# cvsp-lab/ICLR2025_3D-MOM

Hardware: AMD Instinct MI355X
Metric: 4DGS train-steps/sec @200k Gaussians, 960×540, 60 frames; render FPS (higher is better)
Workload: dtype f32; 1 GPU; 200k Gaussians, 60 frames, 960x540, HexPlane on; gaussians=200000, frames=60, width=960, height=540, parallelism=single, ranks_seen=1, gaussians_at_end=200000, steps_replayed_after_overflow=0

## Files before the change

### iclr2025_3d-mom_amd/_native.py

```python
from __future__ import annotations

import ctypes as C
import os
import subprocess

_HERE = os.path.dirname(os.path.abspath(__file__))
LIB_PATH = os.environ.get("MOM4D_LIB") or os.path.join(_HERE, "lib", "libmom4d.so")
_lib = None

MOM_OK, MOM_EINVAL, MOM_ELAUNCH, MOM_ECAPACITY, MOM_EUNAVAILABLE = 0, -1, -2, -3, -4
_ERR = {MOM_EINVAL: "invalid argument", MOM_ELAUNCH: "HIP launch/runtime failure", MOM_ECAPACITY: "scratch too small",
        MOM_EUNAVAILABLE: "run-time dependency missing (librccl)"}
COMM_F32, COMM_I32, COMM_SUM, COMM_MAX = 0, 1, 0, 1


class MomError(RuntimeError):
    pass


GACC_FLOATS = int(os.environ.get("MOM_GACC_FLOATS", "12"))
ABI_VERSION = 8


class MomRasterArgs(C.Structure):
# ... 198 lines not shown
    lib.mom_ssim_forward.argtypes = [i32, i32, i32, vp, vp, vp, vp, vp, vp]
    lib.mom_ssim_forward_slab.argtypes = [i32, i32, i32, sz, i32, i32, i32, i32, vp, vp, vp, vp, vp, vp]
    lib.mom_ssim_backward_slab.argtypes = [i32, i32, i32, sz, vp, vp, vp, vp, C.c_float, vp, vp, vp]
    lib.mom_ssim_backward.argtypes = [i32, i32, i32, vp, vp, vp, vp, C.c_float, vp, vp, vp]
    lib.mom_activations_forward.argtypes = [i32, vp, vp, vp, vp, vp, vp, vp]
    lib.mom_activations_backward.argtypes = [i32, vp, vp, vp, vp, vp, vp, vp, vp, vp, vp]
    lib.mom_image_to_rgb8.argtypes = [i32, i32, i32, vp, vp, vp]
    lib.mom_png_bound.restype = sz
    lib.mom_png_bound.argtypes = [i32, i32, i32]
    lib.mom_png_scratch_bytes.restype = sz
    lib.mom_png_scratch_bytes.argtypes = [i32, i32, i32]
    lib.mom_png_encode.argtypes = [i32, i32, i32, vp, vp, sz, vp, vp, vp]
    lib.mom_png_encode_host.argtypes = [i32, i32, i32, vp, vp, sz, vp]
    lib.mom_png_tables.argtypes = [i32, vp, vp, vp, i32, vp]
    lib.mom_profile_enable.argtypes = [i32, i32]
    lib.mom_profile_read.argtypes = [i32, C.POINTER(C.c_double), C.POINTER(C.c_longlong), i32]
    lib.mom_profile_name.restype = C.c_char_p
    lib.mom_profile_name.argtypes = [i32]
    lib.mom_knn_scratch_bytes.restype = sz
    lib.mom_knn_scratch_bytes.argtypes = [i32]
    lib.mom_knn_mean_dist2.argtypes = [i32, vp, vp, vp, vp]
    return lib


SSIM_SUM_SLOTS = 64
SELECT_MAX_TENSORS = 32


class MomRowSelect(C.Structure):
    _fields_ = [("src", C.c_void_p), ("dst", C.c_void_p), ("row_bytes", C.c_uint)]
# ... 13 lines not shown
    "mom_raster_forward_geometry", "mom_raster_forward_render", "mom_raster_backward", "mom_mark_visible",
    "mom_selftest_wave_sum", "mom_selftest_row_reduce", "mom_hexplane_forward", "mom_hexplane_backward", "mom_hexplane_backward_lines", "mom_adam_step", "mom_l1_loss",
    "mom_plane_regulation", "mom_knn_scratch_bytes", "mom_knn_mean_dist2",
    "mom_profile_enable", "mom_profile_read", "mom_profile_name",
    "mom_morton_order_scratch_bytes", "mom_morton_order", "mom_activations_forward", "mom_activations_backward", "mom_deform_forward", "mom_deform_forward_activated", "mom_deform_backward_scratch_bytes", "mom_deform_backward", "mom_deform_backward_split",
    "mom_ssim_forward", "mom_ssim_backward", "mom_raster_backward_render", "mom_raster_backward_geometry",
    "mom_densify_stats", "mom_select_scratch_bytes", "mom_select_plan", "mom_select_apply",
    "mom_ssim_forward_slab", "mom_ssim_backward_slab",
    "mom_hexplane_backward_scratch_bytes", "mom_hexplane_orders_scratch_bytes", "mom_hexplane_orders", "mom_image_to_rgb8",
    "mom_l1_loss_acc", "mom_plane_regulation_acc", "mom_plane_regulation_grad",
    "mom_deform_field_supported", "mom_deform_field_scratch_bytes", "mom_deform_field_forward",
    "mom_stream_wait_stream", "mom_stream_mark", "mom_stream_wait_mark", "mom_zero_async",
    "mom_comm_available", "mom_comm_last_error", "mom_comm_unique_id", "mom_comm_create", "mom_comm_destroy", "mom_comm_abort",
    "mom_comm_world", "mom_comm_rank", "mom_comm_group_start", "mom_comm_group_end", "mom_comm_all_reduce", "mom_comm_all_gather",
    "mom_comm_reduce_scatter",
    "mom_raster_backward_acc", "mom_raster_backward_geometry_acc",
    "mom_deform_forward_n", "mom_deform_forward_activated_n", "mom_deform_backward_n", "mom_deform_backward_split_n",
    "mom_deform_field16_supported", "mom_deform_field16_scratch_bytes", "mom_deform_field16_forward",
    "mom_densify_scratch_bytes", "mom_densify_plan", "mom_densify_apply",
    "mom_sceneflow_fit_scratch_bytes", "mom_sceneflow_fit", "mom_flow_sample",
    "mom_png_bound", "mom_png_scratch_bytes", "mom_png_encode", "mom_png_encode_host", "mom_png_tables",
]


ABI_STRUCTS = None


def _abi_structs():
    return [("MOM_STRUCT_RASTER_ARGS", MomRasterArgs), ("MOM_STRUCT_RASTER_GRADS", MomRasterGrads),
            ("MOM_STRUCT_RASTER_LAYOUT", MomRasterLayout), ("MOM_STRUCT_HEXPLANE", MomHexPlane),
            ("MOM_STRUCT_ADAM_TENSOR", MomAdamTensor), ("MOM_STRUCT_ROW_SELECT", MomRowSelect),
# ... 74 lines not shown
```

### iclr2025_3d-mom_amd/csrc/mom_common.h

```cpp
#pragma once
#include <hip/hip_runtime.h>
#include <stdint.h>
#include <stddef.h>
#include <stdlib.h>
#include "../../include/mom4d.h"

#define MOM_WAVE 64
#define MOM_ALIGN 256

struct GeomView {
    float4* rec;
    float* cov3D;
    uchar4* clamped;
    float* gacc;
    unsigned long long* reach;
};
struct ImageView {
    uint32_t* hdr;
    uint32_t* tile_counts;
    uint32_t* tile_cursor;
    uint2* ranges;
    uint32_t* n_contrib;
    float* final_T;
    uint32_t* tile_order;
};
struct BinView {
    uint64_t* keys;
    uint32_t* point_list;
};

static inline size_t mom_align_up(size_t x) { return (x + MOM_ALIGN - 1) & ~(size_t)(MOM_ALIGN - 1); }

static inline size_t geom_view(char* base, int P, GeomView* v)
{
    size_t off = 0;
    size_t o_rec = off; off = mom_align_up(off + (size_t)P * 48);
    size_t o_cov = off; off = mom_align_up(off + (size_t)P * 24);
    size_t o_cl = off; off = mom_align_up(off + (size_t)P * 4);
    size_t o_ga = off; off = mom_align_up(off + (size_t)P * MOM_GACC_FLOATS * 4);
// ... 7 lines not shown
    }
    return off + MOM_ALIGN;
}
static inline size_t image_view(char* base, int W, int H, ImageView* v)
{
    const size_t tiles = (size_t)((W + MOM_TILE - 1) / MOM_TILE) * ((H + MOM_TILE - 1) / MOM_TILE);
    const size_t N = (size_t)W * H;
    size_t off = 0;
    size_t o_h = off; off = mom_align_up(off + 64 * 4);
    size_t o_c = off; off = mom_align_up(off + tiles * 4);
    size_t o_u = off; off = mom_align_up(off + tiles * 4);
    size_t o_r = off; off = mom_align_up(off + tiles * 8);
    size_t o_n = off; off = mom_align_up(off + N * 4);
    size_t o_t = off; off = mom_align_up(off + N * 4);
    size_t o_o = off; off = mom_align_up(off + tiles * 4);
    if (v) {
        v->tile_order = (uint32_t*)(base + o_o);
        v->hdr = (uint32_t*)(base + o_h);
        v->tile_counts = (uint32_t*)(base + o_c);
        v->tile_cursor = (uint32_t*)(base + o_u);
        v->ranges = (uint2*)(base + o_r);
        v->n_contrib = (uint32_t*)(base + o_n);
        v->final_T = (float*)(base + o_t);
    }
    return off + MOM_ALIGN;
}
static inline size_t bin_view(char* base, size_t cap, BinView* v)
{
    size_t off = 0;
    size_t o_p = off; off = mom_align_up(off + cap * 4);
    size_t o_k = off; off = mom_align_up(off + cap * 8);
    if (v) {
// ... 117 lines not shown
```

### iclr2025_3d-mom_amd/csrc/raster_api.hip

```cpp
#include "mom_common.h"

int mom_launch_preprocess_fwd(const MomRasterArgs* a, const GeomView& g, int* radii, uint32_t* zero_words, int n_zero, hipStream_t s);
int mom_launch_mark_visible(int P, const float* means3D, const float* view, uint8_t* present, hipStream_t s);
int mom_launch_binning_count(const MomRasterArgs* a, const GeomView& g, const ImageView& im, uint32_t* num_rendered_dev,
                             uint32_t* num_rendered_host, hipStream_t s);
int mom_launch_binning_sort(const MomRasterArgs* a, const GeomView& g, const BinView& b, const ImageView& im, size_t capacity,
                            uint32_t* status_dev, bool render_sorts_small, hipStream_t s);
int mom_launch_render_fwd(const MomRasterArgs* a, const GeomView& g, const BinView& b, const ImageView& im, size_t capacity,
                          float* out_color, float* out_depth, bool sort_small, hipStream_t s);
int mom_launch_render_bwd(const MomRasterArgs* a, const GeomView& g, const BinView& b, const ImageView& im, size_t capacity,
                          const float* dL_dpix, const float* dL_ddepth, hipStream_t s);
int mom_launch_preprocess_bwd(const MomRasterArgs* a, const int* radii, const GeomView& g, const MomRasterGrads* gr, const MomRasterAccum* acc,
                              hipStream_t s);

static int check_args(const MomRasterArgs* a)
{
    if (!a || a->struct_size != sizeof(MomRasterArgs)) return MOM_EINVAL;
    if (a->P < 0 || a->W <= 0 || a->H <= 0) return MOM_EINVAL;
    if (a->tile_row0 < 0 || a->tile_row1 < a->tile_row0 || a->tile_row1 > (a->H + MOM_TILE - 1) / MOM_TILE) return MOM_EINVAL;
    if (a->params_raw && (a->cov3D_precomp || !a->scales || !a->rotations)) return MOM_EINVAL;
    if (a->P == 0) return MOM_OK;
    if (!a->means3D || !a->opacities || !a->viewmatrix || !a->projmatrix || !a->campos || !a->background) return MOM_EINVAL;
    if (!a->shs && !a->colors_precomp) return MOM_EINVAL;
    if (!a->cov3D_precomp && (!a->scales || !a->rotations)) return MOM_EINVAL;
    if (a->shs && !a->colors_precomp && (a->D < 0 || a->D > 3 || a->M < (a->D + 1) * (a->D + 1))) return MOM_EINVAL;
    return MOM_OK;
}

// ... 80 lines not shown
    hipStream_t s = (hipStream_t)stream;
    if (!num_rendered_dev) return MOM_EINVAL;
    if (a->P == 0) {
        if (hipMemsetAsync(num_rendered_dev, 0, 4, s) != hipSuccess) return MOM_ELAUNCH;
        if (num_rendered_host) *num_rendered_host = 0;
        return MOM_OK;
    }
    if (!geom || !image || !radii) return MOM_EINVAL;
    GeomView g; ImageView im;
    geom_view(mom_align_ptr(geom), a->P, &g);
    image_view(mom_align_ptr(image), a->W, a->H, &im);
    const int tiles = ((a->W + MOM_TILE - 1) / MOM_TILE) * ((a->H + MOM_TILE - 1) / MOM_TILE);
    rc = mom_launch_preprocess_fwd(a, g, radii, im.hdr, (int)((im.tile_counts + tiles) - im.hdr), s);
    if (rc) return rc;
    MOM_CHECK_LAUNCH(a, s);
    rc = mom_launch_binning_count(a, g, im, num_rendered_dev, num_rendered_host, s);
    if (rc) return rc;
    MOM_CHECK_LAUNCH(a, s);
    return MOM_OK;
}

int mom_raster_forward_render(const MomRasterArgs* a, void* geom, void* binning, size_t capacity, void* image,
                              float* out_color, float* out_depth, uint32_t* status_dev, mom_stream_t stream)
{
    int rc = check_args(a);
    if (rc) return rc;
    hipStream_t s = (hipStream_t)stream;
    if (!out_color || !out_depth) return MOM_EINVAL;
    const size_t HW = (size_t)a->W * a->H;
    if (a->P == 0) {
        if (hipMemsetAsync(out_color, 0, HW * 12, s) != hipSuccess) return MOM_ELAUNCH;
// ... 89 lines not shown

int mom_raster_backward(const MomRasterArgs* a, const int* radii, void* geom, void* binning, size_t capacity, void* image,
                        const float* dL_dout_color, const float* dL_dout_depth, const MomRasterGrads* gr, mom_stream_t stream)
{
    int rc = check_args(a);
    if (rc) return rc;
    if (a->P == 0) return MOM_OK;
    if (!geom || !binning || !image || !radii || !dL_dout_color) return MOM_EINVAL;
    rc = check_grads(a, gr);
    if (rc) return rc;
    rc = mom_raster_backward_render(a, geom, binning, capacity, image, dL_dout_color, dL_dout_depth, stream);
    if (rc) return rc;
    return mom_raster_backward_geometry(a, radii, geom, gr, stream);
}

int mom_mark_visible(int P, const float* means3D, const float* viewmatrix, const float* projmatrix, uint8_t* present,
                     mom_stream_t stream)
{
    (void)projmatrix;
    if (P < 0) return MOM_EINVAL;
    if (P == 0) return MOM_OK;
    if (!means3D || !viewmatrix || !present) return MOM_EINVAL;
    return mom_launch_mark_visible(P, means3D, viewmatrix, present, (hipStream_t)stream);
}

}
```

### iclr2025_3d-mom_amd/csrc/raster_bin_dev.h

```cpp
#pragma once
#include "mom_common.h"

namespace {

#ifndef MOM_SMALL_RECT
#define MOM_SMALL_RECT 24
#endif
constexpr int kSmallRect = MOM_SMALL_RECT;
constexpr int kMaxLdsTiles = 16384;


struct Reach {
    float cx, cy, a, b, c, bound, inv_a, inv_c;
    int cull;
};
__device__ __forceinline__ bool tile_reached(const Reach& r, int tx, int ty)
{
    if (!r.cull) return true;
    const float xa = (float)(tx * MOM_TILE), ya = (float)(ty * MOM_TILE);
    return mom_rect_reach(r.cx, r.cy, r.a, r.b, r.c, r.bound, r.inv_a, r.inv_c, xa, xa + (float)(MOM_TILE - 1), ya,
                          ya + (float)(MOM_TILE - 1));
}
__device__ __forceinline__ float bcast(float v, int src) { return __int_as_float(__builtin_amdgcn_readlane(__float_as_int(v), src)); }

// ... 133 lines not shown
                if (i1 < n) {
                    uint64_t k0 = k[i0], k1 = k[i1], k2 = ld(i2), k3 = ld(i3);
                    cx(k0, k2); cx(k1, k3);
                    cx(k0, k1); cx(k2, k3);
                    st4(i0, i1, i2, i3, k0, k1, k2, k3);
                }
            }
        }
        if (lj == 0) pairs_pass();
    }
    __syncthreads();
}


constexpr int kRenderSortCap = 1536;
```

### iclr2025_3d-mom_amd/csrc/raster_binning.hip

```cpp
#include "raster_bin_dev.h"

namespace {

constexpr int kSortLdsCap = 8192;
#ifndef MOM_SORT_SMALL
#define MOM_SORT_SMALL 2048
#endif
constexpr int kSortSmallCap = MOM_SORT_SMALL;
constexpr int kOrderBins = 128;

template <class F>
__device__ __forceinline__ void for_each_kept(int x0, int y0, int x1, int y1, int gx, uint32_t payload, uint64_t mask, const Reach& rc, F f)
{
    const int lane = mom_lane();
    const int w = x1 - x0;
    const int cnt = w * (y1 - y0);
    const bool own = cnt <= MOM_WAVE && __popcll(mask) <= kSmallRect;
    if (own && cnt > 0) {
        const float inv_w = __builtin_amdgcn_rcpf((float)w);
        uint64_t m = mask;
        while (m) {
            const int i = __ffsll((long long)m) - 1;
            m &= m - 1;
            const int q = small_div(i, inv_w);
// ... 79 lines not shown
        if (g < P) reach[g] = mask;
    }
    if (LDS_HIST) {
        __syncthreads();
        for (int t = threadIdx.x; t < tiles; t += 256) {
            const uint32_t n = s_cnt[t];
            if (n) atomicAdd(&tile_counts[t], n);
        }
    }
}

__global__ void __launch_bounds__(1024) tile_scan_kernel(int tiles, const uint32_t* __restrict__ tile_counts,
                                                        uint32_t* __restrict__ tile_cursor, uint2* __restrict__ ranges,
                                                        uint32_t* __restrict__ hdr, uint32_t* __restrict__ num_rendered_dev,
                                                        uint32_t* __restrict__ num_rendered_host, int t0, int nt,
                                                        uint32_t* __restrict__ tile_order)
{
    __shared__ uint32_t s_wave[16];
    __shared__ uint32_t s_carry;
    __shared__ uint32_t s_bin[kOrderBins + 1];
    __shared__ uint32_t s_big;
    const int lane = threadIdx.x & 63, wave = threadIdx.x >> 6;
    if (threadIdx.x == 0) s_carry = 0;
    for (int i = threadIdx.x; i <= kOrderBins; i += 1024) s_bin[i] = 0;
    auto bin_of = [&](uint32_t n) { return kOrderBins - 1 - (int)min((uint32_t)(kOrderBins - 1), n >> 5); };
    __syncthreads();
    for (int base = 0; base < tiles; base += 1024) {
        const int t = base + threadIdx.x;
        const uint32_t n = t < tiles ? tile_counts[t] : 0u;
        if (t >= t0 && t < t0 + nt) atomicAdd(&s_bin[bin_of(n) + 1], 1u);
        uint32_t incl = n;
#pragma unroll
        for (int d = 1; d < 64; d <<= 1) {
            const uint32_t o = __shfl_up(incl, d);
            if (lane >= d) incl += o;
        }
        if (lane == 63) s_wave[wave] = incl;
        __syncthreads();
// ... 15 lines not shown
        uint32_t incl = c0 + c1;
#pragma unroll
        for (int d = 1; d < 64; d <<= 1) {
            const uint32_t o = __shfl_up(incl, d);
            if (lane >= d) incl += o;
        }
        const uint32_t excl = incl - (c0 + c1);
        s_bin[2 * lane] = excl;
        s_bin[2 * lane + 1] = excl + c0;
        static_assert(kRenderSortCap % 32 == 0 && kRenderSortCap / 32 < kOrderBins, "class boundary");
        constexpr int kFirstSmall = kOrderBins - kRenderSortCap / 32;
        if (2 * lane == kFirstSmall) s_big = excl;
        if (2 * lane + 1 == kFirstSmall) s_big = excl + c0;
    }
    __syncthreads();
    for (int t = t0 + threadIdx.x; t < t0 + nt; t += 1024) tile_order[atomicAdd(&s_bin[bin_of(tile_counts[t])], 1u)] = (uint32_t)t;
    if (threadIdx.x == 0) {
        hdr[0] = s_carry;
        hdr[3] = (uint32_t)t0;
        hdr[4] = (uint32_t)nt;
        hdr[5] = s_big;
        *num_rendered_dev = s_carry;
        if (num_rendered_host) __hip_atomic_store(num_rendered_host, s_carry, __ATOMIC_RELAXED, __HIP_MEMORY_SCOPE_SYSTEM);
    }
}

template <bool LDS_HIST>
__global__ void __launch_bounds__(256) tile_scatter_kernel(int P, int chunks, int gx, int gy, int ry0, int ry1, int cull, const float4* __restrict__ rec,
                                                          const unsigned long long* __restrict__ reach,
                                                          uint32_t* __restrict__ tile_cursor, uint64_t* __restrict__ keys,
                                                          uint32_t capacity, uint32_t* __restrict__ hdr, uint32_t* __restrict__ sticky,
                                                          uint32_t tag)
// ... 50 lines not shown
    }
    if (overflow) {
        atomicOr(&hdr[1], 1u);
        if (sticky) atomicCAS(sticky, 0u, tag);
    }
}

template <int LO, int CAP>
__global__ void __launch_bounds__(256) tile_sort_kernel(const uint2* __restrict__ ranges, const uint32_t* __restrict__ tile_order,
                                                       uint64_t* __restrict__ keys, uint32_t* __restrict__ point_list, uint32_t capacity,
                                                       const uint32_t* __restrict__ head_count, int nt)
{
    __shared__ uint64_t s_keys[CAP];
    const int limit = head_count ? min((int)*head_count, nt) : nt;
    for (int slot = blockIdx.x; slot < limit; slot += gridDim.x) {
        const uint2 r = ranges[tile_order[slot]];
        uint32_t end = r.y < capacity ? r.y : capacity;
        if (r.x >= end) continue;
        const int n = (int)(end - r.x);
        if (n <= LO || (n > CAP && CAP < kSortLdsCap)) continue;
        uint64_t* gk = keys + r.x;
        __syncthreads();
        if (n <= CAP) {
            for (int i = threadIdx.x; i < n; i += 256) s_keys[i] = gk[i];
            __syncthreads();
            if (n > 1) bitonic_sort<true>(s_keys, n, 256, threadIdx.x);
            for (int i = threadIdx.x; i < n; i += 256) point_list[r.x + i] = (uint32_t)s_keys[i];
        } else {
            __syncthreads();
            bitonic_sort<false>(gk, n, 256, threadIdx.x);
            __threadfence_block();
            for (int i = threadIdx.x; i < n; i += 256) point_list[r.x + i] = (uint32_t)gk[i];
        }
    }
}

}

static int bin_chunks(int P)
{
    const int chunks = (P + 256 * 2048 - 1) / (256 * 2048);
    return chunks < 1 ? 1 : chunks;
}

int mom_launch_binning_count(const MomRasterArgs* a, const GeomView& g, const ImageView& im, uint32_t* num_rendered_dev,
                             uint32_t* num_rendered_host, hipStream_t s)
{
    const int gx = (a->W + MOM_TILE - 1) / MOM_TILE, gy = (a->H + MOM_TILE - 1) / MOM_TILE;
    const int tiles = gx * gy;
    int ry0, ry1;
    mom_tile_rows(a, gy, &ry0, &ry1);
    const int cull = a->keep_all_tiles ? 0 : 1;
    const int chunks = bin_chunks(a->P);
    const int blocks = (a->P + 256 * chunks - 1) / (256 * chunks);
    mom_prof_begin(MOM_P_HIST, s);
    if (tiles <= kMaxLdsTiles)
        hipLaunchKernelGGL(tile_hist_kernel<true>, dim3(blocks), dim3(256), (size_t)tiles * 4, s, a->P, chunks, gx, gy, ry0, ry1, cull,
                           g.rec, im.tile_counts, g.reach);
    else
        hipLaunchKernelGGL(tile_hist_kernel<false>, dim3(blocks), dim3(256), 0, s, a->P, chunks, gx, gy, ry0, ry1, cull, g.rec,
                           im.tile_counts, g.reach);
    mom_prof_end(MOM_P_HIST, s);
    if (hipGetLastError() != hipSuccess) return MOM_ELAUNCH;
    MomProfScope ps(MOM_P_SCAN, s);
    hipLaunchKernelGGL(tile_scan_kernel, dim3(1), dim3(1024), 0, s, tiles, im.tile_counts, im.tile_cursor, im.ranges, im.hdr,
                       num_rendered_dev, num_rendered_host, gx * ry0, gx * (ry1 - ry0), im.tile_order);
    return hipGetLastError() == hipSuccess ? MOM_OK : MOM_ELAUNCH;
}

int mom_launch_binning_sort(const MomRasterArgs* a, const GeomView& g, const BinView& b, const ImageView& im, size_t capacity,
                            uint32_t* status_dev, bool render_sorts_small, hipStream_t s)
{
    const int gx = (a->W + MOM_TILE - 1) / MOM_TILE, gy = (a->H + MOM_TILE - 1) / MOM_TILE;
    const int tiles = gx * gy;
    int ry0, ry1;
    mom_tile_rows(a, gy, &ry0, &ry1);
    const int cull = a->keep_all_tiles ? 0 : 1;
    const int chunks = bin_chunks(a->P);
    const int blocks = (a->P + 256 * chunks - 1) / (256 * chunks);
    const uint32_t cap = capacity > 0xFFFFFFFFull ? 0xFFFFFFFFu : (uint32_t)capacity;
    const uint32_t tag = a->overflow_tag ? a->overflow_tag : 1u;
// ... 25 lines not shown
```

### iclr2025_3d-mom_amd/csrc/raster_render.hip

```cpp
#include "mom_common.h"
#include "raster_bin_dev.h"

namespace {

__device__ __forceinline__ int remap_tile(int b, int nt, int C)
{
    const int full = nt / (8 * C) * (8 * C);
    if (b >= full) return b;
    const int xcd = b & 7, slot = b >> 3, q = slot / C;
    return (q * 8 + xcd) * C + (slot - q * C);
}
static inline int tile_run(int gx) { return gx >= 8 ? gx / 4 : 1; }

template <int CTRL, int ROW_MASK>
__device__ __forceinline__ float dpp_add(float v)
{
    const int o = __builtin_amdgcn_update_dpp(0, __float_as_int(v), CTRL, ROW_MASK, 0xF, false);
    return v + __int_as_float(o);
}
__device__ __forceinline__ float wave_sum(float v)
{
    v = dpp_add<0xB1, 0xF>(v);
    v = dpp_add<0x4E, 0xF>(v);
    v = dpp_add<0x124, 0xF>(v);
// ... 4 lines not shown
}

__device__ __forceinline__ float power_bound(float opacity) { return mom_power_bound(opacity); }

__device__ __forceinline__ float splat_power(const float4 r0, const float4 r1, float pxf, float pyf, float& dx, float& dy)
{
#pragma clang fp contract(off)
    dx = r0.x - pxf;
    dy = r0.y - pyf;
    const float ax = r1.x * dx, cy = r1.z * dy, bx = r1.y * dx;
    const float quad = __builtin_fmaf(cy, dy, ax * dx);
    return __builtin_fmaf(-0.5f, quad, -(bx * dy));
}

constexpr int kFW = 8, kFH = 64 / kFW, kWX = 16 / kFW;
__device__ __forceinline__ uint32_t strip_reach_mask(const float4 r0, const float4 r1, float x0, float y0)
{
    const float a = r1.x, c = r1.z;
    if (!(a > 0.f) || !(c > 0.f)) return 0xFu;
    const float inv_a = __builtin_amdgcn_rcpf(a), inv_c = __builtin_amdgcn_rcpf(c);
    uint32_t m = 0;
#pragma unroll
    for (int w = 0; w < 4; w++) {
        const float xa = x0 + (float)(kFW * (w % kWX)), ya = y0 + (float)(kFH * (w / kWX));
        m |= mom_rect_reach(r0.x, r0.y, a, r1.y, c, r0.w, inv_a, inv_c, xa, xa + (float)(kFW - 1), ya, ya + (float)(kFH - 1)) ? (1u << w) : 0u;
    }
    return m;
}
#define MOM_FWD_WAVES 8
#define MOM_BWD_WAVES 5
struct L1Epilogue {
    const float* target;
    float* grad;
    float* sums;
    float inv_n;
    float* partials;
};
constexpr int kRound = 256, kRoundChunks = kRound / 64;
constexpr int kRoundB = 512, kRoundChunksB = kRoundB / 64;
template <int CHUNKS>
// ... 40 lines not shown
#define BARRIER_T1() do { } while (0)
#define FWD_STAMP(k) do { } while (0)
#define BWD_STAMP(k) do { } while (0)
#define STAMP_ID(arr) do { } while (0)
#define STAMP_LIST(arr, tile, n) do { } while (0)
#define STAMP_EXIT(arr) do { } while (0)
#define STAMP_WAIT() do { } while (0)
#define LANE_HIST(kernel, mask, passed) do { } while (0)
#endif

__global__ void __launch_bounds__(256) __attribute__((amdgpu_waves_per_eu(MOM_FWD_WAVES, MOM_FWD_WAVES)))
render_fwd_kernel(const uint2* __restrict__ ranges, uint32_t* point_list , int W, int H, int gx, int nt, int t0, int run,
                  const uint32_t* __restrict__ tile_order, const uint32_t* __restrict__ order_hdr, const float4* __restrict__ rec, const float* __restrict__ bg, float* __restrict__ final_T,
                  uint32_t* __restrict__ n_contrib, float* __restrict__ out_color, float* __restrict__ out_depth,
                  uint32_t capacity, L1Epilogue l1, const uint64_t* __restrict__ sort_keys, uint32_t* __restrict__ tile_walked,
                  unsigned long long* status_post, uint32_t status_serial)
{
    __shared__ float4 s_rec[kRound * 3];
    __shared__ uint8_t s_mask[kRound];
    __shared__ uint16_t s_lists[4][kRound];
    __shared__ __attribute__((aligned(16))) uint32_t s_live[4];
    FWD_STAMP(0);
    STAMP_ID(g_fwd_stamps);
    const bool ordered = order_hdr[3] == (uint32_t)t0 && order_hdr[4] == (uint32_t)nt;
    const int tile = ordered ? (int)tile_order[blockIdx.x] : t0 + remap_tile(blockIdx.x, nt, run);
    const int tx = tile % gx, ty = tile / gx;

    uint2 range = ranges[tile];
    if (range.y > capacity) range.y = capacity;
    if (range.x > range.y) range.x = range.y;
    int toDo = (int)(range.y - range.x);
    STAMP_WAIT();
    FWD_STAMP(1);
    STAMP_LIST(g_fwd_stamps, tile, toDo);
    const int rounds = (toDo + kRound - 1) / kRound;
    const int list_len = toDo;
    int walked_rounds = rounds;

    static_assert(kRenderSortCap * 8 <= kRound * 3 * 16, "the sort aliases the splat staging area");
    bool have_first = false;
    uint32_t first_id = 0;
    if (sort_keys && toDo > 0 && toDo <= kRenderSortCap) {
        uint64_t* sk = reinterpret_cast<uint64_t*>(s_rec);
        const uint64_t* __restrict__ gk = sort_keys + range.x;
        for (int i = threadIdx.x; i < toDo; i += 256) sk[i] = gk[i];
        __syncthreads();
        if (toDo > 1) bitonic_sort<true>(sk, toDo, 256, (int)threadIdx.x);
        for (int i = threadIdx.x; i < toDo; i += 256) point_list[range.x + i] = (uint32_t)sk[i];
        have_first = true;
        if ((int)threadIdx.x < toDo) first_id = (uint32_t)sk[threadIdx.x];
        __threadfence_block();
        __syncthreads();
    }

    FWD_STAMP(2);
    const int lx = kFW * ((threadIdx.x >> 6) % kWX) + (threadIdx.x & 63) % kFW;
    const int ly = kFH * ((threadIdx.x >> 6) / kWX) + (threadIdx.x & 63) / kFW;
    const int px = tx * MOM_TILE + lx, py = ty * MOM_TILE + ly;
    const bool inside = px < W && py < H;
    const float pxf = (float)px, pyf = (float)py;
    const int wv = threadIdx.x >> 6, lane = threadIdx.x & 63;
    float T = 1.0f;
    uint32_t last_contributor = 0;
    float C0 = 0.f, C1 = 0.f, C2 = 0.f, D = 0.f;
    uint64_t live = __builtin_amdgcn_ballot_w64(inside);

    static_assert(kRound == 256, "one staged splat per thread");
    float4 p0 = make_float4(0.f, 0.f, 0.f, 0.f), p1 = p0, p2 = p0;
    bool pv = false;
    auto fetch = [&](int round) {
        const uint32_t at = range.x + (uint32_t)(round * kRound) + threadIdx.x;
        pv = round < rounds && at < range.y;
        if (pv) {
            const size_t id = (round == 0 && have_first) ? first_id : point_list[at];
// ... 6 lines not shown
    STAMP_WAIT();
    FWD_STAMP(3);
#ifdef FWD_STAMPS
    unsigned long long bar_wait_ = 0;
#endif
    if (lane == 0) s_live[wv] = live != 0;
    for (int i = 0; i < rounds; i++, toDo -= kRound) {
        { BARRIER_T0(); __syncthreads(); BARRIER_T1(); }
        const uint4 lv = *reinterpret_cast<const uint4*>(s_live);
        if (__builtin_amdgcn_readfirstlane((int)(lv.x | lv.y | lv.z | lv.w)) == 0) { walked_rounds = i; break; }
        {
            uint32_t reach = 0;
            if (pv) {
                float4 q0 = p0;
                q0.w = power_bound(p1.w);
                int ox = tx * MOM_TILE, oy = ty * MOM_TILE;
                asm volatile("" : "+s"(ox), "+s"(oy));
                reach = strip_reach_mask(q0, p1, (float)ox, (float)oy);
                s_rec[threadIdx.x * 3 + 0] = q0;
                s_rec[threadIdx.x * 3 + 1] = p1;
                s_rec[threadIdx.x * 3 + 2] = p2;
            }
            s_mask[threadIdx.x] = (uint8_t)reach;
        }
        { BARRIER_T0(); __syncthreads(); BARRIER_T1(); }
        fetch(i + 1);
        int list[kRoundChunks];
        const int n_w = build_wave_list(s_mask, s_lists[wv], wv, lane, list);
#pragma unroll
        for (int c = 0; c < kRoundChunks; c++) {
            const int nk = __builtin_amdgcn_readfirstlane(min(64, n_w - 64 * c));
            for (int k = 0; k < nk; k++) {
                if (live == 0) break;
// ... 23 lines not shown
                    C0 += r2.x * w;
                    C1 += r2.y * w;
                    C2 += r2.z * w;
                    D += r0.z * w;
                    T = test_T;
                    last_contributor = (uint32_t)(i * kRound + j + 1);
                }
            }
        }
        if (lane == 0) s_live[wv] = live != 0;
    }
#ifdef FWD_STAMPS
    if ((threadIdx.x & 63) == 0 && blockIdx.x < kStampGroups) g_fwd_stamps[blockIdx.x * kStampWords + 12 + (threadIdx.x >> 6)] = bar_wait_;
#endif
    FWD_STAMP(4);
    if (threadIdx.x == 0) tile_walked[tile] = (uint32_t)min(list_len, walked_rounds * kRound);
    if (status_post && blockIdx.x == 0 && threadIdx.x == 0)
        __hip_atomic_store(status_post, ((unsigned long long)status_serial << 32) | order_hdr[1], __ATOMIC_RELAXED, __HIP_MEMORY_SCOPE_SYSTEM);
    if (inside) {
        const int pix = py * W + px;
        if (final_T) final_T[pix] = T;
        if (n_contrib) n_contrib[pix] = last_contributor;
        const size_t HW = (size_t)H * W;
        C0 += T * bg[0];
        C1 += T * bg[1];
        C2 += T * bg[2];
        out_color[pix] = C0;
        out_color[HW + pix] = C1;
        out_color[2 * HW + pix] = C2;
        out_depth[pix] = D;
    }
    FWD_STAMP(5);
// ... 7 lines not shown
            for (int k = 0; k < 3; k++) {
                const float d = c[k] - l1.target[k * HW + pix];
                a1 += fabsf(d);
                a2 += d * d;
                l1.grad[k * HW + pix] = d > 0.f ? l1.inv_n : (d < 0.f ? -l1.inv_n : 0.f);
            }
        }
        a1 = wave_sum(a1);
        a2 = wave_sum(a2);
        float* s_sum = reinterpret_cast<float*>(s_lists);
        __syncthreads();
        if (lane == 0) { s_sum[2 * wv] = a1; s_sum[2 * wv + 1] = a2; }
        __syncthreads();
        if (threadIdx.x == 0) {
            const float t1 = (s_sum[0] + s_sum[2]) + (s_sum[4] + s_sum[6]), t2 = (s_sum[1] + s_sum[3]) + (s_sum[5] + s_sum[7]);
            if (l1.partials) {
                reinterpret_cast<float2*>(l1.partials)[tile] = make_float2(t1, t2);
            } else {
                atomicAdd(&l1.sums[0], t1);
                atomicAdd(&l1.sums[1], t2);
            }
        }
    }
    FWD_STAMP(6);
    STAMP_WAIT();
    FWD_STAMP(7);
    STAMP_EXIT(g_fwd_stamps);
}

#define MOM_ROR(d, x, y, n, bank) "v_add_f32_dpp " d ", " x ", " y " row_ror:" n " row_mask:0xf bank_mask:" bank "\n"
#define MOM_QP(d, x, y, perm) "v_add_f32_dpp " d ", " x ", " y " quad_perm:[" perm "] row_mask:0xf bank_mask:0xf\n"
// ... 57 lines not shown

template <bool DEPTH>
__global__ void __launch_bounds__(256) __attribute__((amdgpu_waves_per_eu(MOM_BWD_WAVES, MOM_BWD_WAVES)))
render_bwd_kernel(const uint2* __restrict__ ranges, const uint32_t* __restrict__ point_list, int W, int H, int gx, int nt, int t0, int run,
                  const uint32_t* __restrict__ tile_order, const uint32_t* __restrict__ order_hdr, const float4* __restrict__ rec, const float* __restrict__ bg, const float* __restrict__ final_Ts,
                  const uint32_t* __restrict__ n_contrib, const float* __restrict__ dL_dpixels,
                  const float* __restrict__ dL_dpixel_depths, float* __restrict__ gacc, uint32_t capacity)
{
    __shared__ float4 s_rec[kRoundB * 3];
    __shared__ uint32_t s_id[kRoundB];
    __shared__ uint8_t s_mask[kRoundB];
    __shared__ uint16_t s_lists[4][kRoundB];
    BWD_STAMP(0);
    STAMP_ID(g_bwd_stamps);
    const bool ordered = order_hdr[3] == (uint32_t)t0 && order_hdr[4] == (uint32_t)nt;
    const int tile = ordered ? (int)tile_order[blockIdx.x] : t0 + remap_tile(blockIdx.x, nt, run);
    const int tx = tile % gx, ty = tile / gx;
    const int lx = kFW * ((threadIdx.x >> 6) % kWX) + (threadIdx.x & 63) % kFW;
    const int ly = kFH * ((threadIdx.x >> 6) / kWX) + (threadIdx.x & 63) / kFW;
    const int px = tx * MOM_TILE + lx, py = ty * MOM_TILE + ly;
    const bool inside = px < W && py < H;
    const float pxf = (float)px, pyf = (float)py;
    const int lane = threadIdx.x & 63, wv = threadIdx.x >> 6;

    uint2 range = ranges[tile];
    if (range.y > capacity) range.y = capacity;
    if (range.x > range.y) range.x = range.y;
    int toDo = (int)(range.y - range.x);

    const int pix = inside ? py * W + px : 0;
    const size_t HW = (size_t)H * W;
    const float T_final = inside ? final_Ts[pix] : 0.f;
    float T = T_final;
    uint32_t contributor = (uint32_t)toDo;
    const int last_contributor = inside ? (int)n_contrib[pix] : 0;

// ... 58 lines not shown

    for (int i = 0; i < rounds; i++, toDo -= kRoundB) {
        drain();
        __syncthreads();
#pragma unroll
        for (int sl = 0; sl < kRoundB / 256; sl++) {
            const int slot = threadIdx.x + 256 * sl;
            uint32_t reach = 0;
            const int progress = i * kRoundB + slot;
            if (range.x + progress < range.y) {
                const uint32_t id = point_list[range.y - progress - 1];
                s_id[slot] = id;
                float4 q0 = rec[3 * (size_t)id + 0];
                const float4 q1 = rec[3 * (size_t)id + 1];
                q0.w = power_bound(q1.w);
                reach = strip_reach_mask(q0, q1, (float)(tx * MOM_TILE), (float)(ty * MOM_TILE));
                s_rec[slot * 3 + 0] = q0;
                s_rec[slot * 3 + 1] = q1;
                s_rec[slot * 3 + 2] = rec[3 * (size_t)id + 2];
            }
            s_mask[slot] = (uint8_t)reach;
        }
        __syncthreads();
        int list[kRoundChunksB];
        const int n_w = build_wave_list(s_mask, s_lists[wv], wv, lane, list);
#pragma unroll
        for (int c = 0; c < kRoundChunksB; c++) {
          const int nk = __builtin_amdgcn_readfirstlane(min(64, n_w - 64 * c));
          for (int k = 0; k < nk; k++) {
            const int j = __builtin_amdgcn_readlane(list[c], k);
            contributor = (uint32_t)(toDo - j - 1);
// ... 76 lines not shown
                          float* out_color, float* out_depth, bool sort_small, hipStream_t s)
{
    const int gx = (a->W + MOM_TILE - 1) / MOM_TILE, gy = (a->H + MOM_TILE - 1) / MOM_TILE;
    const uint32_t cap = capacity > 0xFFFFFFFFull ? 0xFFFFFFFFu : (uint32_t)capacity;
    MomProfScope ps(MOM_P_RENDER_FWD, s);
    int ry0, ry1;
    mom_tile_rows(a, gy, &ry0, &ry1);
    const int nt = gx * (ry1 - ry0);
    if (nt == 0) {
        if (a->status_post) hipLaunchKernelGGL(status_post_kernel, dim3(1), dim3(1), 0, s, im.hdr, a->status_post, a->status_serial);
        return hipGetLastError() == hipSuccess ? MOM_OK : MOM_ELAUNCH;
    }
    const float l1_inv_n = 1.0f / (3.0f * (float)a->W * (float)a->H);
    L1Epilogue l1 = {a->l1_target, a->l1_grad, a->l1_sums, a->l1_grad_scale != 0.f ? l1_inv_n * a->l1_grad_scale : l1_inv_n, a->l1_partials};
    if (!l1.grad || (!l1.sums && !l1.partials)) l1.target = nullptr;
    hipLaunchKernelGGL(render_fwd_kernel, dim3(nt), dim3(256), 0, s, im.ranges, b.point_list, a->W, a->H, gx, nt, gx * ry0, tile_run(gx), im.tile_order, im.hdr,
                       g.rec, a->background, a->forward_only ? nullptr : im.final_T, a->forward_only ? nullptr : im.n_contrib, out_color,
                       out_depth, cap, l1, sort_small ? b.keys : nullptr, im.tile_cursor, a->status_post, a->status_serial);
    return hipGetLastError() == hipSuccess ? MOM_OK : MOM_ELAUNCH;
}

int mom_launch_render_bwd(const MomRasterArgs* a, const GeomView& g, const BinView& b, const ImageView& im, size_t capacity,
                          const float* dL_dpix, const float* dL_ddepth, hipStream_t s)
{
    const int gx = (a->W + MOM_TILE - 1) / MOM_TILE, gy = (a->H + MOM_TILE - 1) / MOM_TILE;
    const uint32_t cap = capacity > 0xFFFFFFFFull ? 0xFFFFFFFFu : (uint32_t)capacity;
    if (!a->accum_cleared && hipMemsetAsync(g.gacc, 0, (size_t)a->P * MOM_GACC_FLOATS * 4, s) != hipSuccess) return MOM_ELAUNCH;
    MomProfScope ps(MOM_P_RENDER_BWD, s);
    int ry0, ry1;
    mom_tile_rows(a, gy, &ry0, &ry1);
    const int nt = gx * (ry1 - ry0);
    if (nt == 0) return MOM_OK;
    if (dL_ddepth)
        hipLaunchKernelGGL(render_bwd_kernel<true>, dim3(nt), dim3(256), 0, s, im.ranges, b.point_list, a->W, a->H, gx, nt, gx * ry0, tile_run(gx), im.tile_order, im.hdr,
                           g.rec, a->background, im.final_T, im.n_contrib, dL_dpix, dL_ddepth, g.gacc, cap);
    else
        hipLaunchKernelGGL(render_bwd_kernel<false>, dim3(nt), dim3(256), 0, s, im.ranges, b.point_list, a->W, a->H, gx, nt, gx * ry0, tile_run(gx), im.tile_order, im.hdr,
                           g.rec, a->background, im.final_T, im.n_contrib, dL_dpix, dL_ddepth, g.gacc, cap);
    return hipGetLastError() == hipSuccess ? MOM_OK : MOM_ELAUNCH;
}

#ifdef FWD_STAMPS
extern "C" int mom_debug_fwd_stamps(unsigned long long* host_dst, int groups)
{
    if (groups > kStampGroups) groups = kStampGroups;
    return hipMemcpyFromSymbol(host_dst, HIP_SYMBOL(g_fwd_stamps), (size_t)groups * kStampWords * 8) == hipSuccess ? MOM_OK : MOM_ELAUNCH;
}
extern "C" int mom_debug_lane_hist(unsigned long long* host_dst, int reset)
{
    if (hipMemcpyFromSymbol(host_dst, HIP_SYMBOL(g_lane_hist), sizeof(g_lane_hist)) != hipSuccess) return MOM_ELAUNCH;
    if (reset) { static unsigned long long zero[2 * 7 * 2] = {0}; if (hipMemcpyToSymbol(HIP_SYMBOL(g_lane_hist), zero, sizeof(zero)) != hipSuccess) return MOM_ELAUNCH; }
    return MOM_OK;
// ... 45 lines not shown
```

### include/mom4d.h

```cpp
#ifndef MOM4D_H_INCLUDED
#define MOM4D_H_INCLUDED

#include <stddef.h>
#include <stdint.h>

#ifdef __cplusplus
extern "C" {
#endif

#define MOM_OK 0
#define MOM_EINVAL (-1)
#define MOM_ELAUNCH (-2)
#define MOM_ECAPACITY (-3)
#define MOM_EUNAVAILABLE (-4)

#define MOM_TILE 16

typedef void* mom_stream_t;

#define MOM_ABI_VERSION 8
#ifndef MOM_GACC_FLOATS
#define MOM_GACC_FLOATS 12
#endif
int mom_abi_version(void);
// ... 88 lines not shown
                            const MomRasterGrads* g, const MomRasterAccum* accum, mom_stream_t stream);
int mom_raster_backward_geometry_acc(const MomRasterArgs* a, const int* radii, void* geom, const MomRasterGrads* grads,
                                     const MomRasterAccum* accum, mom_stream_t stream);

int mom_mark_visible(int P, const float* means3D, const float* viewmatrix, const float* projmatrix,
                     uint8_t* present, mom_stream_t stream);

typedef struct MomRasterLayout {
    size_t geom_rec, geom_cov3D, geom_clamped, geom_gacc;
    size_t img_ranges, img_n_contrib, img_final_T, img_tile_counts;
    size_t bin_keys, bin_point_list;
    size_t img_tile_walked;
} MomRasterLayout;
int mom_raster_layout(int P, int W, int H, size_t capacity, MomRasterLayout* out);

size_t mom_knn_scratch_bytes(int P);
int mom_knn_mean_dist2(int P, const float* points , float* mean_dist2 , void* scratch,
                       mom_stream_t stream);

typedef struct MomHexPlane {
    int levels;
    int channels;
    int res[4][4];
    const float* planes[4][6];
    float* grads[4][6];
    float aabb[6];
} MomHexPlane;
int mom_hexplane_forward(const MomHexPlane* hp, int P, const float* xyz, const float* times, float time,
                         const uint32_t* order, float* feat, mom_stream_t stream);
size_t mom_hexplane_backward_scratch_bytes(const MomHexPlane* hp, int P);
// ... 191 lines not shown
```

Before: 1192 steps/s.

## Split heaviest raster tiles into two half-tile blocks in forward and backward

```diff
diff --git a/iclr2025_3d-mom_amd/_native.py b/iclr2025_3d-mom_amd/_native.py
--- a/iclr2025_3d-mom_amd/_native.py
+++ b/iclr2025_3d-mom_amd/_native.py
@@ -236,6 +236,7 @@
     lib.mom_png_encode_host.argtypes = [i32, i32, i32, vp, vp, sz, vp]
     lib.mom_png_tables.argtypes = [i32, vp, vp, vp, i32, vp]
     lib.mom_profile_enable.argtypes = [i32, i32]
+    lib.mom_raster_set_split_above.argtypes = [i32]
     lib.mom_profile_read.argtypes = [i32, C.POINTER(C.c_double), C.POINTER(C.c_longlong), i32]
     lib.mom_profile_name.restype = C.c_char_p
     lib.mom_profile_name.argtypes = [i32]
@@ -279,7 +280,7 @@
     "mom_comm_available", "mom_comm_last_error", "mom_comm_unique_id", "mom_comm_create", "mom_comm_destroy", "mom_comm_abort",
     "mom_comm_world", "mom_comm_rank", "mom_comm_group_start", "mom_comm_group_end", "mom_comm_all_reduce", "mom_comm_all_gather",
     "mom_comm_reduce_scatter",
-    "mom_raster_backward_acc", "mom_raster_backward_geometry_acc",
+    "mom_raster_backward_acc", "mom_raster_backward_geometry_acc", "mom_raster_set_split_above",
     "mom_deform_forward_n", "mom_deform_forward_activated_n", "mom_deform_backward_n", "mom_deform_backward_split_n",
     "mom_deform_field16_supported", "mom_deform_field16_scratch_bytes", "mom_deform_field16_forward",
     "mom_densify_scratch_bytes", "mom_densify_plan", "mom_densify_apply",
diff --git a/iclr2025_3d-mom_amd/csrc/mom_common.h b/iclr2025_3d-mom_amd/csrc/mom_common.h
--- a/iclr2025_3d-mom_amd/csrc/mom_common.h
+++ b/iclr2025_3d-mom_amd/csrc/mom_common.h
@@ -8,6 +8,7 @@
 #define MOM_WAVE 64
 #define MOM_ALIGN 256
 
+#define MOM_MAX_SPLIT 256
 struct GeomView {
     float4* rec;
     float* cov3D;
@@ -23,6 +24,8 @@
     uint32_t* n_contrib;
     float* final_T;
     uint32_t* tile_order;
+    uint32_t* split_ticket;
+    unsigned long long* split_sums;
 };
 struct BinView {
     uint64_t* keys;
@@ -60,8 +63,12 @@
     size_t o_n = off; off = mom_align_up(off + N * 4);
     size_t o_t = off; off = mom_align_up(off + N * 4);
     size_t o_o = off; off = mom_align_up(off + tiles * 4);
+    size_t o_s = off; off = mom_align_up(off + MOM_MAX_SPLIT * 4);
+    size_t o_q = off; off = mom_align_up(off + MOM_MAX_SPLIT * 8);
     if (v) {
         v->tile_order = (uint32_t*)(base + o_o);
+        v->split_ticket = (uint32_t*)(base + o_s);
+        v->split_sums = (unsigned long long*)(base + o_q);
         v->hdr = (uint32_t*)(base + o_h);
         v->tile_counts = (uint32_t*)(base + o_c);
         v->tile_cursor = (uint32_t*)(base + o_u);
diff --git a/iclr2025_3d-mom_amd/csrc/raster_api.hip b/iclr2025_3d-mom_amd/csrc/raster_api.hip
--- a/iclr2025_3d-mom_amd/csrc/raster_api.hip
+++ b/iclr2025_3d-mom_amd/csrc/raster_api.hip
@@ -3,7 +3,7 @@
 int mom_launch_preprocess_fwd(const MomRasterArgs* a, const GeomView& g, int* radii, uint32_t* zero_words, int n_zero, hipStream_t s);
 int mom_launch_mark_visible(int P, const float* means3D, const float* view, uint8_t* present, hipStream_t s);
 int mom_launch_binning_count(const MomRasterArgs* a, const GeomView& g, const ImageView& im, uint32_t* num_rendered_dev,
-                             uint32_t* num_rendered_host, hipStream_t s);
+                             uint32_t* num_rendered_host, uint32_t split_above, hipStream_t s);
 int mom_launch_binning_sort(const MomRasterArgs* a, const GeomView& g, const BinView& b, const ImageView& im, size_t capacity,
                             uint32_t* status_dev, bool render_sorts_small, hipStream_t s);
 int mom_launch_render_fwd(const MomRasterArgs* a, const GeomView& g, const BinView& b, const ImageView& im, size_t capacity,
@@ -12,6 +12,9 @@
                           const float* dL_dpix, const float* dL_ddepth, hipStream_t s);
 int mom_launch_preprocess_bwd(const MomRasterArgs* a, const int* radii, const GeomView& g, const MomRasterGrads* gr, const MomRasterAccum* acc,
                               hipStream_t s);
+
+constexpr int kSplitAboveDefault = 896;
+static int g_split_above = kSplitAboveDefault;
 
 static int check_args(const MomRasterArgs* a)
 {
@@ -122,7 +125,7 @@
     rc = mom_launch_preprocess_fwd(a, g, radii, im.hdr, (int)((im.tile_counts + tiles) - im.hdr), s);
     if (rc) return rc;
     MOM_CHECK_LAUNCH(a, s);
-    rc = mom_launch_binning_count(a, g, im, num_rendered_dev, num_rendered_host, s);
+    rc = mom_launch_binning_count(a, g, im, num_rendered_dev, num_rendered_host, (uint32_t)__atomic_load_n(&g_split_above, __ATOMIC_RELAXED), s);
     if (rc) return rc;
     MOM_CHECK_LAUNCH(a, s);
     return MOM_OK;
@@ -242,6 +245,11 @@
     return mom_raster_backward_geometry(a, radii, geom, gr, stream);
 }
 
+int mom_raster_set_split_above(int n)
+{
+    return __atomic_exchange_n(&g_split_above, n < 0 ? kSplitAboveDefault : n, __ATOMIC_RELAXED);
+}
+
 int mom_mark_visible(int P, const float* means3D, const float* viewmatrix, const float* projmatrix, uint8_t* present,
                      mom_stream_t stream)
 {
diff --git a/iclr2025_3d-mom_amd/csrc/raster_bin_dev.h b/iclr2025_3d-mom_amd/csrc/raster_bin_dev.h
--- a/iclr2025_3d-mom_amd/csrc/raster_bin_dev.h
+++ b/iclr2025_3d-mom_amd/csrc/raster_bin_dev.h
@@ -171,3 +171,25 @@
 
 
 constexpr int kRenderSortCap = 1536;
+
+constexpr int kMaxSplit = MOM_MAX_SPLIT;
+constexpr uint32_t kSplitBit = 0x80000000u, kTileMask = 0x7FFFFFFFu;
+__device__ __forceinline__ bool launch_slot(const uint32_t* __restrict__ tile_order, bool ordered, int nt, int block, int& order_pos, uint32_t& entry, int& half)
+{
+    half = -1;
+    entry = 0;
+    if (block < kMaxSplit) {
+        order_pos = block;
+        if (!ordered || block >= nt) return false;
+        entry = tile_order[block];
+        if (!(entry & kSplitBit)) return false;
+        half = 1;
+        return true;
+    }
+    order_pos = block - kMaxSplit;
+    if (ordered) {
+        entry = tile_order[order_pos];
+        if (entry & kSplitBit) half = 0;
+    }
+    return true;
+}
diff --git a/iclr2025_3d-mom_amd/csrc/raster_binning.hip b/iclr2025_3d-mom_amd/csrc/raster_binning.hip
--- a/iclr2025_3d-mom_amd/csrc/raster_binning.hip
+++ b/iclr2025_3d-mom_amd/csrc/raster_binning.hip
@@ -117,14 +117,18 @@
                                                         uint32_t* __restrict__ tile_cursor, uint2* __restrict__ ranges,
                                                         uint32_t* __restrict__ hdr, uint32_t* __restrict__ num_rendered_dev,
                                                         uint32_t* __restrict__ num_rendered_host, int t0, int nt,
-                                                        uint32_t* __restrict__ tile_order)
+                                                        uint32_t* __restrict__ tile_order, uint32_t split_above,
+                                                        uint32_t* __restrict__ split_ticket, unsigned long long* __restrict__ split_sums)
 {
     __shared__ uint32_t s_wave[16];
     __shared__ uint32_t s_carry;
     __shared__ uint32_t s_bin[kOrderBins + 1];
     __shared__ uint32_t s_big;
+    __shared__ uint32_t s_split;
     const int lane = threadIdx.x & 63, wave = threadIdx.x >> 6;
-    if (threadIdx.x == 0) s_carry = 0;
+    if (threadIdx.x == 0) s_carry = s_split = 0;
+    static_assert(kMaxSplit <= 1024, "one ticket word per thread");
+    if (threadIdx.x < kMaxSplit) { split_ticket[threadIdx.x] = 0; split_sums[threadIdx.x] = 0; }
     for (int i = threadIdx.x; i <= kOrderBins; i += 1024) s_bin[i] = 0;
     auto bin_of = [&](uint32_t n) { return kOrderBins - 1 - (int)min((uint32_t)(kOrderBins - 1), n >> 5); };
     __syncthreads();
@@ -170,8 +174,16 @@
         if (2 * lane + 1 == kFirstSmall) s_big = excl + c0;
     }
     __syncthreads();
-    for (int t = t0 + threadIdx.x; t < t0 + nt; t += 1024) tile_order[atomicAdd(&s_bin[bin_of(tile_counts[t])], 1u)] = (uint32_t)t;
+    for (int t = t0 + threadIdx.x; t < t0 + nt; t += 1024) {
+        const uint32_t n = tile_counts[t];
+        const uint32_t pos = atomicAdd(&s_bin[bin_of(n)], 1u);
+        const bool split = split_above != 0 && n > split_above && pos < (uint32_t)kMaxSplit;
+        tile_order[pos] = (uint32_t)t | (split ? kSplitBit : 0u);
+        if (split) atomicAdd(&s_split, 1u);
+    }
+    __syncthreads();
     if (threadIdx.x == 0) {
+        hdr[6] = s_split;
         hdr[0] = s_carry;
         hdr[3] = (uint32_t)t0;
         hdr[4] = (uint32_t)nt;
@@ -252,7 +264,7 @@
     __shared__ uint64_t s_keys[CAP];
     const int limit = head_count ? min((int)*head_count, nt) : nt;
     for (int slot = blockIdx.x; slot < limit; slot += gridDim.x) {
-        const uint2 r = ranges[tile_order[slot]];
+        const uint2 r = ranges[tile_order[slot] & kTileMask];
         uint32_t end = r.y < capacity ? r.y : capacity;
         if (r.x >= end) continue;
         const int n = (int)(end - r.x);
@@ -282,7 +294,7 @@
 }
 
 int mom_launch_binning_count(const MomRasterArgs* a, const GeomView& g, const ImageView& im, uint32_t* num_rendered_dev,
-                             uint32_t* num_rendered_host, hipStream_t s)
+                             uint32_t* num_rendered_host, uint32_t split_above, hipStream_t s)
 {
     const int gx = (a->W + MOM_TILE - 1) / MOM_TILE, gy = (a->H + MOM_TILE - 1) / MOM_TILE;
     const int tiles = gx * gy;
@@ -302,7 +314,7 @@
     if (hipGetLastError() != hipSuccess) return MOM_ELAUNCH;
     MomProfScope ps(MOM_P_SCAN, s);
     hipLaunchKernelGGL(tile_scan_kernel, dim3(1), dim3(1024), 0, s, tiles, im.tile_counts, im.tile_cursor, im.ranges, im.hdr,
-                       num_rendered_dev, num_rendered_host, gx * ry0, gx * (ry1 - ry0), im.tile_order);
+                       num_rendered_dev, num_rendered_host, gx * ry0, gx * (ry1 - ry0), im.tile_order, split_above, im.split_ticket, im.split_sums);
     return hipGetLastError() == hipSuccess ? MOM_OK : MOM_ELAUNCH;
 }
 
diff --git a/iclr2025_3d-mom_amd/csrc/raster_render.hip b/iclr2025_3d-mom_amd/csrc/raster_render.hip
--- a/iclr2025_3d-mom_amd/csrc/raster_render.hip
+++ b/iclr2025_3d-mom_amd/csrc/raster_render.hip
@@ -42,7 +42,19 @@
 }
 
 constexpr int kFW = 8, kFH = 64 / kFW, kWX = 16 / kFW;
-__device__ __forceinline__ uint32_t strip_reach_mask(const float4 r0, const float4 r1, float x0, float y0)
+struct Footprint {
+    int y0;
+    int fh;
+};
+__device__ __forceinline__ Footprint make_footprint(int half) { return half < 0 ? Footprint{0, kFH} : Footprint{half * (MOM_TILE / 2), kFH / 2}; }
+__device__ __forceinline__ bool footprint_pixel(const Footprint& f, int tid, int& lx, int& ly)
+{
+    const int wv = tid >> 6, lane = tid & 63;
+    lx = kFW * (wv % kWX) + lane % kFW;
+    ly = f.y0 + f.fh * (wv / kWX) + lane / kFW;
+    return lane / kFW < f.fh;
+}
+__device__ __forceinline__ uint32_t strip_reach_mask(const float4 r0, const float4 r1, float x0, float y0, int fh)
 {
     const float a = r1.x, c = r1.z;
     if (!(a > 0.f) || !(c > 0.f)) return 0xFu;
@@ -50,8 +62,8 @@
     uint32_t m = 0;
 #pragma unroll
     for (int w = 0; w < 4; w++) {
-        const float xa = x0 + (float)(kFW * (w % kWX)), ya = y0 + (float)(kFH * (w / kWX));
-        m |= mom_rect_reach(r0.x, r0.y, a, r1.y, c, r0.w, inv_a, inv_c, xa, xa + (float)(kFW - 1), ya, ya + (float)(kFH - 1)) ? (1u << w) : 0u;
+        const float xa = x0 + (float)(kFW * (w % kWX)), ya = y0 + (float)(fh * (w / kWX));
+        m |= mom_rect_reach(r0.x, r0.y, a, r1.y, c, r0.w, inv_a, inv_c, xa, xa + (float)(kFW - 1), ya, ya + (float)(fh - 1)) ? (1u << w) : 0u;
     }
     return m;
 }
@@ -122,7 +134,7 @@
                   const uint32_t* __restrict__ tile_order, const uint32_t* __restrict__ order_hdr, const float4* __restrict__ rec, const float* __restrict__ bg, float* __restrict__ final_T,
                   uint32_t* __restrict__ n_contrib, float* __restrict__ out_color, float* __restrict__ out_depth,
                   uint32_t capacity, L1Epilogue l1, const uint64_t* __restrict__ sort_keys, uint32_t* __restrict__ tile_walked,
-                  unsigned long long* status_post, uint32_t status_serial)
+                  uint32_t* __restrict__ split_ticket, unsigned long long* __restrict__ split_sums, unsigned long long* status_post, uint32_t status_serial)
 {
     __shared__ float4 s_rec[kRound * 3];
     __shared__ uint8_t s_mask[kRound];
@@ -131,8 +143,12 @@
     FWD_STAMP(0);
     STAMP_ID(g_fwd_stamps);
     const bool ordered = order_hdr[3] == (uint32_t)t0 && order_hdr[4] == (uint32_t)nt;
-    const int tile = ordered ? (int)tile_order[blockIdx.x] : t0 + remap_tile(blockIdx.x, nt, run);
+    int order_pos, half;
+    uint32_t entry;
+    if (!launch_slot(tile_order, ordered, nt, (int)blockIdx.x, order_pos, entry, half)) return;
+    const int tile = ordered ? (int)(entry & kTileMask) : t0 + remap_tile(order_pos, nt, run);
     const int tx = tile % gx, ty = tile / gx;
+    const Footprint fp = make_footprint(half);
 
     uint2 range = ranges[tile];
     if (range.y > capacity) range.y = capacity;
@@ -162,10 +178,10 @@
     }
 
     FWD_STAMP(2);
-    const int lx = kFW * ((threadIdx.x >> 6) % kWX) + (threadIdx.x & 63) % kFW;
-    const int ly = kFH * ((threadIdx.x >> 6) / kWX) + (threadIdx.x & 63) / kFW;
+    int lx, ly;
+    const bool has_pixel = footprint_pixel(fp, (int)threadIdx.x, lx, ly);
     const int px = tx * MOM_TILE + lx, py = ty * MOM_TILE + ly;
-    const bool inside = px < W && py < H;
+    const bool inside = has_pixel && px < W && py < H;
     const float pxf = (float)px, pyf = (float)py;
     const int wv = threadIdx.x >> 6, lane = threadIdx.x & 63;
     float T = 1.0f;
@@ -202,9 +218,9 @@
             if (pv) {
                 float4 q0 = p0;
                 q0.w = power_bound(p1.w);
-                int ox = tx * MOM_TILE, oy = ty * MOM_TILE;
-                asm volatile("" : "+s"(ox), "+s"(oy));
-                reach = strip_reach_mask(q0, p1, (float)ox, (float)oy);
+                int ox = tx * MOM_TILE, oy = ty * MOM_TILE + fp.y0, fh = fp.fh;
+                asm volatile("" : "+s"(ox), "+s"(oy), "+s"(fh));
+                reach = strip_reach_mask(q0, p1, (float)ox, (float)oy, fh);
                 s_rec[threadIdx.x * 3 + 0] = q0;
                 s_rec[threadIdx.x * 3 + 1] = p1;
                 s_rec[threadIdx.x * 3 + 2] = p2;
@@ -258,8 +274,19 @@
     if ((threadIdx.x & 63) == 0 && blockIdx.x < kStampGroups) g_fwd_stamps[blockIdx.x * kStampWords + 12 + (threadIdx.x >> 6)] = bar_wait_;
 #endif
     FWD_STAMP(4);
-    if (threadIdx.x == 0) tile_walked[tile] = (uint32_t)min(list_len, walked_rounds * kRound);
-    if (status_post && blockIdx.x == 0 && threadIdx.x == 0)
+    if (threadIdx.x == 0) {
+        const uint32_t walked = (uint32_t)min(list_len, walked_rounds * kRound);
+        if (half < 0) {
+            tile_walked[tile] = walked;
+        } else {
+            const uint32_t other = atomicExch(&split_ticket[order_pos], walked + 1u);
+            if (other) {
+                tile_walked[tile] = max(other - 1u, walked);
+                atomicExch(&split_ticket[order_pos], 0u);
+            }
+        }
+    }
+    if (status_post && blockIdx.x == kMaxSplit && threadIdx.x == 0)
         __hip_atomic_store(status_post, ((unsigned long long)status_serial << 32) | order_hdr[1], __ATOMIC_RELAXED, __HIP_MEMORY_SCOPE_SYSTEM);
     if (inside) {
         const int pix = py * W + px;
@@ -297,7 +324,15 @@
         __syncthreads();
         if (threadIdx.x == 0) {
             const float t1 = (s_sum[0] + s_sum[2]) + (s_sum[4] + s_sum[6]), t2 = (s_sum[1] + s_sum[3]) + (s_sum[5] + s_sum[7]);
-            if (l1.partials) {
+            if (l1.partials && half >= 0) {
+                const unsigned long long mine = ((unsigned long long)__float_as_uint(t2) << 32) | (__float_as_uint(t1) | 0x80000000u);
+                const unsigned long long other = atomicExch(&split_sums[order_pos], mine);
+                if (other) {
+                    const float o1 = __uint_as_float((uint32_t)other & 0x7FFFFFFFu), o2 = __uint_as_float((uint32_t)(other >> 32));
+                    reinterpret_cast<float2*>(l1.partials)[tile] = make_float2(t1 + o1, t2 + o2);
+                    atomicExch(&split_sums[order_pos], 0ull);
+                }
+            } else if (l1.partials) {
                 reinterpret_cast<float2*>(l1.partials)[tile] = make_float2(t1, t2);
             } else {
                 atomicAdd(&l1.sums[0], t1);
@@ -385,12 +420,16 @@
     BWD_STAMP(0);
     STAMP_ID(g_bwd_stamps);
     const bool ordered = order_hdr[3] == (uint32_t)t0 && order_hdr[4] == (uint32_t)nt;
-    const int tile = ordered ? (int)tile_order[blockIdx.x] : t0 + remap_tile(blockIdx.x, nt, run);
+    int order_pos, half;
+    uint32_t entry;
+    if (!launch_slot(tile_order, ordered, nt, (int)blockIdx.x, order_pos, entry, half)) return;
+    const int tile = ordered ? (int)(entry & kTileMask) : t0 + remap_tile(order_pos, nt, run);
     const int tx = tile % gx, ty = tile / gx;
-    const int lx = kFW * ((threadIdx.x >> 6) % kWX) + (threadIdx.x & 63) % kFW;
-    const int ly = kFH * ((threadIdx.x >> 6) / kWX) + (threadIdx.x & 63) / kFW;
+    const Footprint fp = make_footprint(half);
+    int lx, ly;
+    const bool has_pixel = footprint_pixel(fp, (int)threadIdx.x, lx, ly);
     const int px = tx * MOM_TILE + lx, py = ty * MOM_TILE + ly;
-    const bool inside = px < W && py < H;
+    const bool inside = has_pixel && px < W && py < H;
     const float pxf = (float)px, pyf = (float)py;
     const int lane = threadIdx.x & 63, wv = threadIdx.x >> 6;
 
@@ -479,7 +518,7 @@
                 float4 q0 = rec[3 * (size_t)id + 0];
                 const float4 q1 = rec[3 * (size_t)id + 1];
                 q0.w = power_bound(q1.w);
-                reach = strip_reach_mask(q0, q1, (float)(tx * MOM_TILE), (float)(ty * MOM_TILE));
+                reach = strip_reach_mask(q0, q1, (float)(tx * MOM_TILE), (float)(ty * MOM_TILE + fp.y0), fp.fh);
                 s_rec[slot * 3 + 0] = q0;
                 s_rec[slot * 3 + 1] = q1;
                 s_rec[slot * 3 + 2] = rec[3 * (size_t)id + 2];
@@ -586,9 +625,9 @@
     const float l1_inv_n = 1.0f / (3.0f * (float)a->W * (float)a->H);
     L1Epilogue l1 = {a->l1_target, a->l1_grad, a->l1_sums, a->l1_grad_scale != 0.f ? l1_inv_n * a->l1_grad_scale : l1_inv_n, a->l1_partials};
     if (!l1.grad || (!l1.sums && !l1.partials)) l1.target = nullptr;
-    hipLaunchKernelGGL(render_fwd_kernel, dim3(nt), dim3(256), 0, s, im.ranges, b.point_list, a->W, a->H, gx, nt, gx * ry0, tile_run(gx), im.tile_order, im.hdr,
+    hipLaunchKernelGGL(render_fwd_kernel, dim3(nt + kMaxSplit), dim3(256), 0, s, im.ranges, b.point_list, a->W, a->H, gx, nt, gx * ry0, tile_run(gx), im.tile_order, im.hdr,
                        g.rec, a->background, a->forward_only ? nullptr : im.final_T, a->forward_only ? nullptr : im.n_contrib, out_color,
-                       out_depth, cap, l1, sort_small ? b.keys : nullptr, im.tile_cursor, a->status_post, a->status_serial);
+                       out_depth, cap, l1, sort_small ? b.keys : nullptr, im.tile_cursor, im.split_ticket, im.split_sums, a->status_post, a->status_serial);
     return hipGetLastError() == hipSuccess ? MOM_OK : MOM_ELAUNCH;
 }
 
@@ -604,10 +643,10 @@
     const int nt = gx * (ry1 - ry0);
     if (nt == 0) return MOM_OK;
     if (dL_ddepth)
-        hipLaunchKernelGGL(render_bwd_kernel<true>, dim3(nt), dim3(256), 0, s, im.ranges, b.point_list, a->W, a->H, gx, nt, gx * ry0, tile_run(gx), im.tile_order, im.hdr,
+        hipLaunchKernelGGL(render_bwd_kernel<true>, dim3(nt + kMaxSplit), dim3(256), 0, s, im.ranges, b.point_list, a->W, a->H, gx, nt, gx * ry0, tile_run(gx), im.tile_order, im.hdr,
                            g.rec, a->background, im.final_T, im.n_contrib, dL_dpix, dL_ddepth, g.gacc, cap);
     else
-        hipLaunchKernelGGL(render_bwd_kernel<false>, dim3(nt), dim3(256), 0, s, im.ranges, b.point_list, a->W, a->H, gx, nt, gx * ry0, tile_run(gx), im.tile_order, im.hdr,
+        hipLaunchKernelGGL(render_bwd_kernel<false>, dim3(nt + kMaxSplit), dim3(256), 0, s, im.ranges, b.point_list, a->W, a->H, gx, nt, gx * ry0, tile_run(gx), im.tile_order, im.hdr,
                            g.rec, a->background, im.final_T, im.n_contrib, dL_dpix, dL_ddepth, g.gacc, cap);
     return hipGetLastError() == hipSuccess ? MOM_OK : MOM_ELAUNCH;
 }
diff --git a/include/mom4d.h b/include/mom4d.h
--- a/include/mom4d.h
+++ b/include/mom4d.h
@@ -126,6 +126,8 @@
 } MomRasterLayout;
 int mom_raster_layout(int P, int W, int H, size_t capacity, MomRasterLayout* out);
 
+int mom_raster_set_split_above(int n);
+
 size_t mom_knn_scratch_bytes(int P);
 int mom_knn_mean_dist2(int P, const float* points , float* mean_dist2 , void* scratch,
                        mom_stream_t stream);
```

Measured after the change: 1193 steps/s, median of 3. About the same (+0.1%).
